# PaddlePaddle/Parakeet

Hardware: NVIDIA H100
Metric: audio-samples/sec (higher is better)
Workload: dtype bf16x3 (split-bf16 operands, fp32 accumulate; fp32-grade, 1e-3 parity)

## Files before the change

### parakeet_b200/csrc/pwg_fc.cu

```cuda
#include <stdlib.h>
#include <string.h>

#include <algorithm>

#include "pk_host.h"
#include "pk_sm90.cuh"

namespace pk {
namespace fc {

constexpr int kPwgR = 64;
constexpr int kPwgG = 128;
constexpr int kATile = 128 * kSwizzleBytes;
constexpr int kQTile = 64 * kSwizzleBytes;
constexpr int kConsumerThreads = 256;
constexpr int kThreads = kConsumerThreads + 128;
constexpr int kFcG1Chunks = 4;
constexpr int kFcStages = 6;
constexpr int kFcStageBytes = 2 * kQTile;
constexpr int kFcUBytes = 2 * 64 * 32;
constexpr int kFcPBytes = 2 * 128 * 32;
constexpr int kFcW1Bytes = 3 * 2 * kATile;
constexpr int kFcW2Bytes = 2 * kATile;
constexpr int kFcSmem = kFcW1Bytes + kFcW2Bytes + kFcStages * kFcStageBytes + 1024 + 256;
static_assert(kFcUBytes + kFcPBytes <= kFcStageBytes, "the conditioning operands share one ring stage");
static_assert(kFcSmem <= 227 * 1024, "shared memory budget");

struct FcLayerArgs {
  int batch, t, dil, hop;
  int u_period, u_start_row, u_end_base;
  int p_row0;
  const int32_t* lens;
  float gate_c[128];
  float out_b[64];
  float k_a, k_g;
  float* skip;
  int skip_init;
};

__device__ __forceinline__ float ex2_approx(float x) {
  float y;
  asm("ex2.approx.ftz.f32 %0, %1;" : "=f"(y) : "f"(x));
  return y;
}
__device__ __forceinline__ float rcp_approx(float x) {
  float y;
  asm("rcp.approx.ftz.f32 %0, %1;" : "=f"(y) : "f"(x));
  return y;
}
__device__ __forceinline__ void split2(float a, float b, uint32_t& hi, uint32_t& lo) {
  const __nv_bfloat162 h = __floats2bfloat162_rn(a, b);
  hi = *reinterpret_cast<const uint32_t*>(&h);
  const float ra = a - __uint_as_float(hi << 16);
  const float rb = b - __uint_as_float(hi & 0xffff0000u);
  const __nv_bfloat162 l = __floats2bfloat162_rn(ra, rb);
  lo = *reinterpret_cast<const uint32_t*>(&l);
}

struct FcTileIter {
  int idx, step, tiles_per_b, total, t;
  const int32_t* lens;
  __device__ FcTileIter(const FcLayerArgs& p)
      : idx(static_cast<int>(blockIdx.x) - static_cast<int>(gridDim.x)), step(gridDim.x),
        tiles_per_b((p.t + 255) >> 8), total(((p.t + 255) >> 8) * p.batch * 2), t(p.t), lens(p.lens) {}
  __device__ bool next(int& b, int& m0, int& half) {
    for (;;) {
      idx += step;
      if (idx >= total) return false;
      const int w = idx >> 1;
      half = idx & 1;
      b = w / tiles_per_b;
      m0 = (w % tiles_per_b) * 256;
      const int len = lens ? min(__ldg(lens + b), t) : t;
      if (m0 < len) return true;
    }
  }
};

__global__ void __launch_bounds__(kThreads, 1)
pwg_layer_fc_kernel(const __grid_constant__ CUtensorMap tm_x, const __grid_constant__ CUtensorMap tm_u,
                    const __grid_constant__ CUtensorMap tm_p,
                    const __grid_constant__ CUtensorMap tm_w1_hi, const __grid_constant__ CUtensorMap tm_w1_lo,
                    const __grid_constant__ CUtensorMap tm_w2_hi, const __grid_constant__ CUtensorMap tm_w2_lo,
                    const __grid_constant__ CUtensorMap tm_y, const FcLayerArgs p) {
  extern __shared__ uint8_t smem_raw[];
  const uint32_t smem = (smem_u32(smem_raw) + 1023u) & ~1023u;
  const uint32_t w1 = smem;
  const uint32_t w2 = w1 + kFcW1Bytes;
  const uint32_t ring = w2 + kFcW2Bytes;
  const uint32_t bars = ring + kFcStages * kFcStageBytes;
  const uint32_t full_bar = bars;
  const uint32_t empty_bar = full_bar + 8 * kFcStages;
  const uint32_t w_bar = empty_bar + 8 * kFcStages;

  const int warp = threadIdx.x >> 5;
  const int lane = threadIdx.x & 31;

  if (threadIdx.x == kConsumerThreads) {
    tma_prefetch_desc(&tm_x); tma_prefetch_desc(&tm_u); tma_prefetch_desc(&tm_p);
    tma_prefetch_desc(&tm_w1_hi); tma_prefetch_desc(&tm_w1_lo); tma_prefetch_desc(&tm_w2_hi); tma_prefetch_desc(&tm_w2_lo);
    tma_prefetch_desc(&tm_y);
    for (int s = 0; s < kFcStages; ++s) { mbar_init_a(full_bar + 8 * s, 1); mbar_init_a(empty_bar + 8 * s, 4); }
    mbar_init_a(w_bar, 1);
    fence_barrier_init();
  }
  __syncthreads();

  if (warp >= kConsumerThreads / 32) {
    setmaxnreg_dec<40>();
    if (warp == kConsumerThreads / 32 && lane == 0) {
      mbar_arrive_expect_tx_a(w_bar, kFcW1Bytes + kFcW2Bytes);
      for (int j = 0; j < 3; ++j) {
        tma_load_3d_a(w1 + j * 2 * kATile, &tm_w1_hi, w_bar, j * kChunkK, 0, 0);
        tma_load_3d_a(w1 + j * 2 * kATile + kATile, &tm_w1_lo, w_bar, j * kChunkK, 0, 0);
      }
      tma_load_3d_a(w2, &tm_w2_hi, w_bar, 0, 0, 0);
      tma_load_3d_a(w2 + kATile, &tm_w2_lo, w_bar, 0, 0, 0);
      uint32_t it = 0;
      FcTileIter ti(p);
      int b, m0, half;
      while (ti.next(b, m0, half)) {
        const int mh = m0 + 128 * half;
        const int len = p.lens ? min(__ldg(p.lens + b), p.t) : p.t;
        const int m1 = ((len - 128) >> 7) << 7;
        const int urow = mh == 0 ? p.u_start_row
                         : (mh + 128 > len - 128) ? p.u_end_base + 384 * b + min(mh - m1, 256)
                                                  : mh % p.u_period;
        const int j0 = (m0 / p.hop - 2) & ~7;
        for (int wg = 0; wg < 2; ++wg) {
          const int rows = min(64, p.t - (mh + 64 * wg));
          if (!p.skip_init && rows > 0)
            bulk_prefetch_l2(p.skip + (static_cast<long long>(b) * p.t + mh + 64 * wg) * 64, rows * 64 * 4);
          for (int j = 0; j < kFcG1Chunks; ++j, ++it) {
            const int s = it % kFcStages;
            mbar_wait_a(empty_bar + 8 * s, ((it / kFcStages) & 1) ^ 1);
            const uint32_t st = ring + s * kFcStageBytes;
            const uint32_t fb = full_bar + 8 * s;
            if (j == 2) {
              mbar_arrive_expect_tx_a(fb, kFcUBytes + kFcPBytes);
              tma_load_4d_a(st, &tm_u, fb, 0, urow + 64 * wg, 0, 0);
              tma_load_4d_a(st + kFcUBytes, &tm_p, fb, j0, p.p_row0, b, 0);
            } else {
              mbar_arrive_expect_tx_a(fb, kFcStageBytes);
              const int wj = j == 0 ? 0 : j == 1 ? 2 : 1;
              tma_load_4d_a(st, &tm_x, fb, 0, mh + 64 * wg + (wj - 1) * p.dil, b, 0);
            }
          }
        }
      }
    }
  } else {
    setmaxnreg_inc<232>();
    const int wg = warp >> 2;
    const int rl = 16 * (warp & 3) + (lane >> 2);
    const int cq = 2 * (lane & 3);
    const float kSqrtHalf = 0.70710678118654752440f;
    mbar_wait_a(w_bar, 0);
    uint32_t it = wg * kFcG1Chunks;
    FcTileIter ti(p);
    int b, m0, half;
    bool more = ti.next(b, m0, half);
    bool first = true;
    while (more) {
      const int mh = m0 + 128 * half;
      float acc1[64], acc2[64];
      if (wg == 1 || !first) named_bar_sync(1 + wg, kConsumerThreads);
      first = false;
#pragma unroll
      for (int j = 0; j < kFcG1Chunks; ++j) {
        const int s = (it + j) % kFcStages;
        mbar_wait_a(full_bar + 8 * s, ((it + j) / kFcStages) & 1);
        const uint32_t st = ring + s * kFcStageBytes;
        wgmma_fence();
        if (j == 2) {
          const uint64_t a_hi = make_smem_desc_sw32(st), a_lo = make_smem_desc_sw32(st + kFcUBytes / 2);
          const uint64_t b_hi = make_smem_desc_sw32(st + kFcUBytes), b_lo = make_smem_desc_sw32(st + kFcUBytes + kFcPBytes / 2);
          wgmma_ss_n128(acc1, a_hi, b_hi, 1);
          wgmma_ss_n128(acc1, a_lo, b_hi, 1);
          wgmma_ss_n128(acc1, a_hi, b_lo, 1);
        } else {
          const int wj = j == 0 ? 0 : j == 1 ? 2 : 1;
          const uint64_t a_hi = make_smem_desc_sw128(st), a_lo = make_smem_desc_sw128(st + kQTile);
          const uint64_t b_hi = make_smem_desc_sw128(w1 + wj * 2 * kATile), b_lo = make_smem_desc_sw128(w1 + wj * 2 * kATile + kATile);
#pragma unroll
          for (int k = 0; k < 4; ++k) {
            wgmma_ss_n128(acc1, a_hi + desc_kstep(k), b_hi + desc_kstep(k), !(j == 0 && k == 0));
            wgmma_ss_n128(acc1, a_lo + desc_kstep(k), b_hi + desc_kstep(k), 1);
            wgmma_ss_n128(acc1, a_hi + desc_kstep(k), b_lo + desc_kstep(k), 1);
          }
        }
        wgmma_commit();
        if (j == kFcG1Chunks - 1) {
#pragma unroll
          for (int jj = 0; jj < 8; ++jj) {
#pragma unroll
            for (int hh = 0; hh < 2; ++hh) {
              const int r = rl + 8 * hh;
              const uint32_t off = r * kSwizzleBytes + ((((8 * jj + cq) >> 3) ^ (r & 7)) << 4) + (cq & 7) * 2;
              const uint32_t xh = lds_u32(st + off), xl = lds_u32(st + kQTile + off);
              acc2[4 * jj + 2 * hh] = 0.f;
              acc2[4 * jj + 2 * hh + 1] = 0.f;
              acc2[32 + 4 * jj + 2 * hh] = __uint_as_float(xh << 16) + __uint_as_float(xl << 16);
              acc2[32 + 4 * jj + 2 * hh + 1] = __uint_as_float(xh & 0xffff0000u) + __uint_as_float(xl & 0xffff0000u);
            }
          }
        }
        if (j > 0) {
          wgmma_wait<1>();
          __syncwarp();
          if (lane == 0) mbar_arrive_a(empty_bar + 8 * ((it + j - 1) % kFcStages));
        }
      }
      wgmma_wait<0>();
      reg_fence(acc1);
      const int cs = (it + kFcG1Chunks - 1) % kFcStages;
      const uint32_t ystage = ring + cs * kFcStageBytes;
      it += 2 * kFcG1Chunks;
      int nb, nm0, nhalf;
      const bool next = ti.next(nb, nm0, nhalf);
      if (wg == 0 || next) named_bar_arrive(2 - wg, kConsumerThreads);
      uint32_t zh[16], zl[16];
#pragma unroll
      for (int jj = 0; jj < 8; ++jj) {
        float z[4];
#pragma unroll
        for (int e = 0; e < 4; ++e) {
          const int c = 8 * jj + cq + (e & 1);
          const float e1 = ex2_approx(fminf(fmaf(acc1[4 * jj + e], p.k_a, p.gate_c[c]), 60.f));
          const float e2 = ex2_approx(fmaf(acc1[32 + 4 * jj + e], p.k_g, p.gate_c[64 + c]));
          const float t1 = 1.f + e1;
          z[e] = (1.f - e1) * rcp_approx(fmaf(t1, e2, t1));
        }
        split2(z[0], z[1], zh[2 * jj], zl[2 * jj]);
        split2(z[2], z[3], zh[2 * jj + 1], zl[2 * jj + 1]);
      }
      const uint64_t b2_hi = make_smem_desc_sw128(w2), b2_lo = make_smem_desc_sw128(w2 + kATile);
      wgmma_fence();
#pragma unroll
      for (int k = 0; k < 4; ++k) {
        const uint32_t ah[4] = {zh[4 * k], zh[4 * k + 1], zh[4 * k + 2], zh[4 * k + 3]};
        const uint32_t al[4] = {zl[4 * k], zl[4 * k + 1], zl[4 * k + 2], zl[4 * k + 3]};
        wgmma_rs_n128(acc2, ah, b2_hi + desc_kstep(k), 1);
        wgmma_rs_n128(acc2, al, b2_hi + desc_kstep(k), 1);
        wgmma_rs_n128(acc2, ah, b2_lo + desc_kstep(k), 1);
      }
      wgmma_commit();
      wgmma_wait<0>();
      reg_fence(acc2);
      const int len = p.lens ? min(__ldg(p.lens + b), p.t) : p.t;
#pragma unroll
      for (int hh = 0; hh < 2; ++hh) {
        const int r = rl + 8 * hh;
        const bool live = mh + wg * 64 + r < len;
#pragma unroll
        for (int jj = 0; jj < 8; ++jj) {
          const int c = 8 * jj + cq;
          const float y0 = live ? (acc2[32 + 4 * jj + 2 * hh] + p.out_b[c]) * kSqrtHalf : 0.f;
          const float y1 = live ? (acc2[32 + 4 * jj + 2 * hh + 1] + p.out_b[c + 1]) * kSqrtHalf : 0.f;
          uint32_t oh, ol;
          split2(y0, y1, oh, ol);
          const uint32_t off = r * kSwizzleBytes + (((c >> 3) ^ (r & 7)) << 4) + (cq & 7) * 2;
          sts_u32(ystage + off, oh);
          sts_u32(ystage + kQTile + off, ol);
        }
      }
      fence_proxy_async_all();
      named_bar_sync(3 + wg, 128);
      const bool store_lane = (threadIdx.x & 127) == 0;
      if (store_lane) {
        tma_store_4d_a(&tm_y, ystage, 0, mh + wg * 64, b, 0);
        bulk_commit();
      }
#pragma unroll
      for (int hh = 0; hh < 2; ++hh) {
        const int trow = mh + wg * 64 + rl + 8 * hh;
        if (trow < p.t) {
          const long long row_off = (static_cast<long long>(b) * p.t + trow) * 64;
#pragma unroll
          for (int jj = 0; jj < 8; ++jj) {
            float* d2 = p.skip + row_off + 8 * jj + cq;
            const float s0 = acc2[4 * jj + 2 * hh], s1 = acc2[4 * jj + 2 * hh + 1];
            if (p.skip_init) *reinterpret_cast<float2*>(d2) = make_float2(s0, s1);
            else asm volatile("red.global.add.v2.f32 [%0], {%1, %2};" ::"l"(d2), "f"(s0), "f"(s1) : "memory");
          }
        }
      }
      if (store_lane) {
        bulk_wait_read<0>();
#pragma unroll
        for (int w = 0; w < 4; ++w) mbar_arrive_a(empty_bar + 8 * cs);
      }
      b = nb; m0 = nm0; half = nhalf; more = next;
    }
  }
}

}
}

extern "C" int pk_pwg_residual_layer_fc(const pk_pwg_layer_fc_args* a, pk_stream_t stream) {
  using namespace pk;
  using namespace pk::fc;
  PK_CHECK_ARG(a != nullptr, "args is NULL");
  PK_CHECK_ARG(a->batch > 0 && a->t > 0 && a->dilation >= 1 && a->hop >= 256, "bad batch/t/dilation/hop (hop must be >= 256)");
  PK_CHECK_ARG(a->x_hi && a->x_lo && a->y_hi && a->y_lo && a->u_hi && a->u_lo && a->p_hi && a->p_lo && a->w1_hi && a->w1_lo &&
               a->w2_hi && a->w2_lo && a->bias1 && a->bias2 && a->skip, "NULL pointer in pk_pwg_layer_fc_args");
  PK_CHECK_ARG(a->x_hi != a->y_hi, "layer output must not alias its input");
  PK_CHECK_ARG(a->u_period > 0 && (a->u_period % 128) == 0 && a->u_start_row >= a->u_period && a->u_end_base >= a->u_start_row + 128 &&
               a->u_rows >= a->u_end_base + 384 * a->batch, "bad compact band table layout");
  PK_CHECK_ARG(a->p_rows > 0 && a->p_row0 >= 0 && a->p_row0 + 128 <= a->p_rows && (a->p_ld % 8) == 0 && a->p_ld >= 64 && a->p_frames > 0 &&
               a->p_frames <= a->p_ld, "bad P plane geometry");
  CUtensorMap tx, tu, tp, tw1_hi, tw1_lo, tw2_hi, tw2_lo, ty;
  int rc;
  const uint64_t T = a->t, B = a->batch;
  if ((rc = encode_tmap_bf16_planes(&tx, a->x_hi, a->x_lo, kPwgR, T, B, kPwgR, T * kPwgR, 64))) return rc;
  if ((rc = encode_tmap_bf16_planes(&ty, a->y_hi, a->y_lo, kPwgR, T, B, kPwgR, T * kPwgR, 64))) return rc;
  if ((rc = encode_tmap_bf16_planes(&tu, a->u_hi, a->u_lo, 64, a->u_rows, 1, 64, 0, 64, 16))) return rc;
  const uint64_t prow = a->p_rows, pld = a->p_ld;
  if ((rc = encode_tmap_bf16_planes(&tp, a->p_hi, a->p_lo, pld, prow, B, pld, prow * pld, 128, 16))) return rc;
  const uint64_t k1 = 5 * kChunkK;
  if ((rc = encode_tmap_bf16_3d(&tw1_hi, a->w1_hi, 3 * kChunkK, kPwgG, 1, k1, k1 * kPwgG, 128))) return rc;
  if ((rc = encode_tmap_bf16_3d(&tw1_lo, a->w1_lo, 3 * kChunkK, kPwgG, 1, k1, k1 * kPwgG, 128))) return rc;
  if ((rc = encode_tmap_bf16_3d(&tw2_hi, a->w2_hi, 64, 128, 1, 64, 0, 128))) return rc;
  if ((rc = encode_tmap_bf16_3d(&tw2_lo, a->w2_lo, 64, 128, 1, 64, 0, 128))) return rc;
  static bool attr_set = false;
  if (!attr_set) {
    PK_CHECK_CUDA(cudaFuncSetAttribute(pwg_layer_fc_kernel, cudaFuncAttributeMaxDynamicSharedMemorySize, kFcSmem));
    attr_set = true;
  }
  FcLayerArgs p;
  p.batch = a->batch; p.t = a->t; p.dil = a->dilation; p.hop = a->hop;
  p.u_period = a->u_period; p.u_start_row = a->u_start_row; p.u_end_base = a->u_end_base;
  p.p_row0 = a->p_row0;
  p.lens = a->lens; p.skip = a->skip; p.skip_init = a->skip_init;
  constexpr float kLog2e = 1.4426950408889634f;
  p.k_a = -2.f * kLog2e; p.k_g = -kLog2e;
  for (int i = 0; i < 64; ++i) {
    p.gate_c[i] = -2.f * kLog2e * a->bias1[i];
    p.gate_c[64 + i] = -kLog2e * a->bias1[64 + i];
    p.out_b[i] = a->bias2[64 + i];
  }
  const cudaStream_t st = static_cast<cudaStream_t>(stream);
  const int tiles = ((a->t + 255) / 256) * 2 * a->batch;
  const int grid = std::min(tiles, sm_count());
  pwg_layer_fc_kernel<<<grid, kThreads, kFcSmem, static_cast<cudaStream_t>(stream)>>>(tx, tu, tp, tw1_hi, tw1_lo, tw2_hi, tw2_lo, ty, p);
  PK_CHECK_CUDA(cudaGetLastError());
  count_launch();
  return PK_OK;
}
```

Measured before the change: 65.11 million.

## Use dedicated output staging and vectorize skip reductions with warp shuffles

```diff
diff --git a/parakeet_b200/csrc/pwg_fc.cu b/parakeet_b200/csrc/pwg_fc.cu
--- a/parakeet_b200/csrc/pwg_fc.cu
+++ b/parakeet_b200/csrc/pwg_fc.cu
@@ -16,13 +16,14 @@
 constexpr int kConsumerThreads = 256;
 constexpr int kThreads = kConsumerThreads + 128;
 constexpr int kFcG1Chunks = 4;
-constexpr int kFcStages = 6;
+constexpr int kFcStages = 4;
 constexpr int kFcStageBytes = 2 * kQTile;
 constexpr int kFcUBytes = 2 * 64 * 32;
 constexpr int kFcPBytes = 2 * 128 * 32;
 constexpr int kFcW1Bytes = 3 * 2 * kATile;
 constexpr int kFcW2Bytes = 2 * kATile;
-constexpr int kFcSmem = kFcW1Bytes + kFcW2Bytes + kFcStages * kFcStageBytes + 1024 + 256;
+constexpr int kFcYBytes = 2 * kFcStageBytes;
+constexpr int kFcSmem = kFcW1Bytes + kFcW2Bytes + kFcStages * kFcStageBytes + kFcYBytes + 1024 + 256;
 static_assert(kFcUBytes + kFcPBytes <= kFcStageBytes, "the conditioning operands share one ring stage");
 static_assert(kFcSmem <= 227 * 1024, "shared memory budget");
 
@@ -88,7 +89,8 @@
   const uint32_t w1 = smem;
   const uint32_t w2 = w1 + kFcW1Bytes;
   const uint32_t ring = w2 + kFcW2Bytes;
-  const uint32_t bars = ring + kFcStages * kFcStageBytes;
+  const uint32_t ystage0 = ring + kFcStages * kFcStageBytes;
+  const uint32_t bars = ystage0 + kFcYBytes;
   const uint32_t full_bar = bars;
   const uint32_t empty_bar = full_bar + 8 * kFcStages;
   const uint32_t w_bar = empty_bar + 8 * kFcStages;
@@ -214,7 +216,9 @@
       wgmma_wait<0>();
       reg_fence(acc1);
       const int cs = (it + kFcG1Chunks - 1) % kFcStages;
-      const uint32_t ystage = ring + cs * kFcStageBytes;
+      __syncwarp();
+      if (lane == 0) mbar_arrive_a(empty_bar + 8 * cs);
+      const uint32_t ystage = ystage0 + wg * kFcStageBytes;
       it += 2 * kFcG1Chunks;
       int nb, nm0, nhalf;
       const bool next = ti.next(nb, nm0, nhalf);
@@ -271,25 +275,24 @@
         tma_store_4d_a(&tm_y, ystage, 0, mh + wg * 64, b, 0);
         bulk_commit();
       }
-#pragma unroll
-      for (int hh = 0; hh < 2; ++hh) {
-        const int trow = mh + wg * 64 + rl + 8 * hh;
-        if (trow < p.t) {
-          const long long row_off = (static_cast<long long>(b) * p.t + trow) * 64;
-#pragma unroll
-          for (int jj = 0; jj < 8; ++jj) {
-            float* d2 = p.skip + row_off + 8 * jj + cq;
-            const float s0 = acc2[4 * jj + 2 * hh], s1 = acc2[4 * jj + 2 * hh + 1];
-            if (p.skip_init) *reinterpret_cast<float2*>(d2) = make_float2(s0, s1);
-            else asm volatile("red.global.add.v2.f32 [%0], {%1, %2};" ::"l"(d2), "f"(s0), "f"(s1) : "memory");
+      {
+        const bool odd = lane & 1;
+        const int trow = mh + wg * 64 + rl + (odd ? 8 : 0);
+        const long long row_off = (static_cast<long long>(b) * p.t + trow) * 64 + (cq & 4);
+#pragma unroll
+        for (int jj = 0; jj < 8; ++jj) {
+          const float g0 = odd ? acc2[4 * jj] : acc2[4 * jj + 2], g1 = odd ? acc2[4 * jj + 1] : acc2[4 * jj + 3];
+          const float r0 = __shfl_xor_sync(0xffffffffu, g0, 1), r1 = __shfl_xor_sync(0xffffffffu, g1, 1);
+          const float4 v = odd ? make_float4(r0, r1, acc2[4 * jj + 2], acc2[4 * jj + 3])
+                               : make_float4(acc2[4 * jj], acc2[4 * jj + 1], r0, r1);
+          if (trow < p.t) {
+            float* d4 = p.skip + row_off + 8 * jj;
+            if (p.skip_init) *reinterpret_cast<float4*>(d4) = v;
+            else asm volatile("red.global.add.v4.f32 [%0], {%1, %2, %3, %4};" ::"l"(d4), "f"(v.x), "f"(v.y), "f"(v.z), "f"(v.w) : "memory");
           }
         }
       }
-      if (store_lane) {
-        bulk_wait_read<0>();
-#pragma unroll
-        for (int w = 0; w < 4; ++w) mbar_arrive_a(empty_bar + 8 * cs);
-      }
+      if (store_lane) bulk_wait_read<0>();
       b = nb; m0 = nm0; half = nhalf; more = next;
     }
   }
```

Result: no change. 64.90 million (median of 6 runs) (-0.3%).
